# xyg-coder/min_llm_inference

Measured on AMD Instinct MI355X. Metric: decode tokens/sec (whole node) on synthetic batch, higher is better.
Workload: dtype bf16; 1 GPU; c4: paged KV decode step (attention + greedy decoder head, n_new=0), 1024 rows/GPU, emb_dim 512, max_seq 4096, lengths U[1024,1550], bf16 pages and weights, fp32 accumulate; lean composition: what the layers run -- no scores / probabilities / emb_score materialised, chunks merged inside the scan launch; rows_per_gpu=1024, rows_total=1024, emb_dim=512, max_seq=4096, n_vocab=1024, parallelism=row-sharded replicas x1, all-gather of token ids

## Files before the change

min_llm_inference_amd/csrc/attention_scan.hip:

```cpp
#include <string>

#include "device_common.hpp"
#include "scan_plan.hpp"

namespace mli {

constexpr int kScanThreads = 256;
constexpr int kScanWaves = kScanThreads / kWave;
constexpr int kMaxChunkTokens = 1024;
constexpr int kMinChunkTokens = 64;

void set_bf16_native_mfma(int v);
void set_scan_merge(int v);
void set_gemm_panel(int v);
void set_scan_stream(int v);
void set_scan_stream_min(int v);
void set_stream_dyn_pct(int v);
void set_stream_granule(int v);
void set_scan_resident_mib(int v);
void set_gemm_split(int v);
void set_bf16_split(int v);
void set_prefill_fused(int v);
void set_gemm_tall_tiles(int v);
void set_fill_compact(int v);
void set_latest_compact(int v);

static thread_local int g_chunk_tokens = 0;
static thread_local int g_nt_loads = 2;
static thread_local int g_row_order = 1;

constexpr int kQktUnits = 16384;
constexpr int kSvUnits = 2048;
constexpr int kSvMaxChunkTokens = 512;

static int pick_chunk_tokens(int n_batch, int n_sequence, int min_units = kQktUnits, int max_ct = kMaxChunkTokens) {
    if (g_chunk_tokens) return g_chunk_tokens;
    int ct = max_ct;
    while (ct > kMinChunkTokens && (int64_t)n_batch * ceil_div_i(n_sequence, ct) < min_units) ct >>= 1;
    return ct;
}

template <bool NT>
__global__ __launch_bounds__(kScanThreads) void qkt_paged_kernel(
    const float* __restrict__ q, const float* const* __restrict__ page_table,
    const int* __restrict__ lengths, float* __restrict__ qkt, int S, int D, int ct, SoftmaxStats st) {
    extern __shared__ __align__(16) unsigned char smem_raw[];
    __shared__ float2 wave_stats[kScanWaves];
    const int b = blockIdx.x;
    const int L = lengths[b];
    const int s0 = blockIdx.y * ct;
    if (s0 >= L) return;

    const int W = S / kPage;
    const int D4 = D >> 2;
    const int s1 = min(s0 + ct, L);
    const int npages = (s1 - s0 + kPage - 1) / kPage;

    float4* q_sh = reinterpret_cast<float4*>(smem_raw);
    const float** ptr_sh = reinterpret_cast<const float**>(smem_raw + (size_t)D4 * 16);

    const float4* q4 = reinterpret_cast<const float4*>(q + (int64_t)b * D);
    for (int i = threadIdx.x; i < D4; i += kScanThreads) q_sh[i] = q4[i];
    for (int i = threadIdx.x; i < npages; i += kScanThreads)
        ptr_sh[i] = page_table[(int64_t)b * W + s0 / kPage + i];
    __syncthreads();

    const int lane = threadIdx.x & (kWave - 1);
    const int wave = threadIdx.x >> 6;
    const float scale = sqrtf((float)D);
    const int nj = (D4 + kWave - 1) / kWave;
    constexpr int TB = 8;

    float run_m = -INFINITY, run_l = 0.f;
    for (int pi = wave; pi < npages; pi += kScanWaves) {
        const float* page = wave_uniform(ptr_sh[pi]);
        const float* krow = page + D;
        float acc[16];
#pragma unroll
        for (int t = 0; t < 16; ++t) acc[t] = 0.f;
        for (int j = 0; j < nj; ++j) {
            const int i4 = lane + j * kWave;
            if (i4 < D4) {
                const float4 qv = q_sh[i4];
                const unsigned voff = (unsigned)i4 * 16u;
#pragma unroll
                for (int h = 0; h < 16 / TB; ++h) {
                    float4 kv[TB];
#pragma unroll
                    for (int t = 0; t < TB; ++t) {
                        const float* trow = krow + (int64_t)(h * TB + t) * 3 * D;
                        kv[t] = ldg4<NT>(byte_offset(trow, voff));
                    }
#pragma unroll
                    for (int t = 0; t < TB; ++t) acc[h * TB + t] = dot4(qv, kv[t], acc[h * TB + t]);
                }
            }
        }
        const float tot = wave_reduce16(acc, lane);
        const int s = s0 + pi * kPage + (lane >> 2);
        const bool writer = (lane & 3) == 0 && s < L;
        const float score = tot / scale;
        if (writer) qkt[(int64_t)b * S + s] = score;
        if (st.stats != nullptr) stats_accumulate(score, writer, run_m, run_l);
    }
    if (st.stats != nullptr) {
        if (lane == 0) wave_stats[wave] = make_float2(run_m, run_l);
        __syncthreads();
        if (threadIdx.x == 0) {
            float m = -INFINITY;
            for (int w = 0; w < kScanWaves; ++w) m = fmaxf(m, wave_stats[w].x);
            float l = 0.f;
            for (int w = 0; w < kScanWaves; ++w)
                if (wave_stats[w].x != -INFINITY) l += wave_stats[w].y * expf(wave_stats[w].x - m);
            st.stats[(int64_t)b * st.per_row + blockIdx.y] = make_float2(m, l);
        }
    }
}

__global__ __launch_bounds__(kScanThreads) void qkt_naive_kernel(
    const float* __restrict__ q, const float* __restrict__ kt, const int* __restrict__ lengths,
    float* __restrict__ qkt, int S, int D, SoftmaxStats st) {
    extern __shared__ __align__(16) unsigned char smem_raw[];
    float4 (*red)[kWave] = reinterpret_cast<float4 (*)[kWave]>(smem_raw);
    float* q_sh = reinterpret_cast<float*>(smem_raw + sizeof(float4) * kScanWaves * kWave);
    const int b = blockIdx.x;
    const int L = lengths[b];
    const int s0 = blockIdx.y * 256;
    if (s0 >= L) return;
    for (int i = threadIdx.x; i < D; i += kScanThreads) q_sh[i] = q[(int64_t)b * D + i];
    __syncthreads();

    const int lane = threadIdx.x & (kWave - 1);
    const int wave = threadIdx.x >> 6;
    const int s = s0 + lane * 4;
    const bool in_row = s < S && s < L;
    const float* base = kt + (int64_t)b * D * S + s;
    const int d_per_wave = (D + kScanWaves - 1) / kScanWaves;
    const int d0 = wave * d_per_wave;
    const int d1 = min(d0 + d_per_wave, D);
    float4 acc = make_float4(0.f, 0.f, 0.f, 0.f);
    if (in_row) {
        int d = d0;
        for (; d + 8 <= d1; d += 8) {
            float4 kv[8];
#pragma unroll
            for (int u = 0; u < 8; ++u) kv[u] = *reinterpret_cast<const float4*>(base + (int64_t)(d + u) * S);
#pragma unroll
            for (int u = 0; u < 8; ++u) axpy4(q_sh[d + u], kv[u], acc);
        }
        for (; d < d1; ++d) axpy4(q_sh[d], *reinterpret_cast<const float4*>(base + (int64_t)d * S), acc);
    }
    red[wave][lane] = acc;
    __syncthreads();
    if (wave == 0) {
        float v[4] = {0.f, 0.f, 0.f, 0.f};
        if (in_row) {
            float4 r = red[0][lane];
#pragma unroll
            for (int w = 1; w < kScanWaves; ++w) {
                r.x += red[w][lane].x; r.y += red[w][lane].y; r.z += red[w][lane].z; r.w += red[w][lane].w;
            }
            const float scale = sqrtf((float)D);
            float* out = qkt + (int64_t)b * S + s;
            v[0] = r.x / scale; v[1] = r.y / scale; v[2] = r.z / scale; v[3] = r.w / scale;
            if (s + 4 <= L) {
                *reinterpret_cast<float4*>(out) = make_float4(v[0], v[1], v[2], v[3]);
            } else {
                for (int u = 0; u < 4; ++u) if (s + u < L) out[u] = v[u];
            }
        }
        if (st.stats != nullptr) {
            float m = -INFINITY, l = 0.f;
#pragma unroll
            for (int u = 0; u < 4; ++u) stats_accumulate(v[u], in_row && s + u < L, m, l);
// ... 307 lines not shown
#undef MLI_QKT_LAUNCH
    return launch_status();
}

int launch_qkt_paged(const float* q, const float* const* page_table, const int* lengths, float* qkt,
                     int B, int S, int D, hipStream_t st) {
    return launch_qkt_paged_stats(q, page_table, lengths, qkt, B, S, D, kNoStats, st);
}

int launch_qkt_naive_stats(const float* q, const float* kt, const int* lengths, float* qkt, int B, int S, int D,
                           SoftmaxStats stats, hipStream_t st) {
    if (S % 4 != 0 || B <= 0) return MLI_ERR_BAD_ARG;
    hipLaunchKernelGGL(qkt_naive_kernel, dim3(B, ceil_div_i(S, 256)), dim3(kScanThreads),
                       sizeof(float4) * kScanWaves * kWave + (size_t)D * 4, st, q, kt, lengths, qkt, S, D, stats);
    return launch_status();
}

int launch_qkt_naive(const float* q, const float* kt, const int* lengths, float* qkt, int B, int S, int D,
                     hipStream_t st) {
    return launch_qkt_naive_stats(q, kt, lengths, qkt, B, S, D, kNoStats, st);
}

int launch_softmax(float* qkt, const int* lengths, int B, int S, hipStream_t st) {
    if (S % 4 != 0 || B <= 0) return MLI_ERR_BAD_ARG;
    hipLaunchKernelGGL(softmax_lengths_kernel, dim3(B), dim3(kScanThreads), 0, st, qkt, lengths, B, S);
    return launch_status();
}

int launch_softmax_v_naive(const float* probs, const float* v_cache, const int* lengths, float* out,
                           int B, int S, int D, void* ws, size_t ws_bytes, hipStream_t st) {
    if (B <= 0 || S <= 0 || D <= 0) return MLI_ERR_BAD_ARG;
    float* p = const_cast<float*>(probs);
    if (D % 4 == 0) return launch_softmax_v_impl<4, false>(p, v_cache, lengths, out, B, S, D, ws, ws_bytes, kNoStats, st);
    return launch_softmax_v_impl<1, false>(p, v_cache, lengths, out, B, S, D, ws, ws_bytes, kNoStats, st);
}

int launch_softmax_v_paged(const float* probs, const float* const* page_table, const int* lengths, float* out,
                           int B, int S, int D, void* ws, size_t ws_bytes, hipStream_t st) {
    if (S % kPage != 0 || D % 4 != 0 || B <= 0) return MLI_ERR_BAD_ARG;
    return launch_softmax_v_impl<4, true>(const_cast<float*>(probs), page_table, lengths, out, B, S, D, ws, ws_bytes,
                                          kNoStats, st);
}

static thread_local int g_fused_softmax = -1;

static bool can_fuse(int B, int S, int stats_chunk, void* ws, size_t ws_bytes) {
    const bool want = g_fused_softmax == 1 || (g_fused_softmax < 0 && (int64_t)B * S <= (1 << 20));
    return want && ws != nullptr && ws_bytes >= stats_region_bytes(B, S) && ceil_div_i(S, stats_chunk) <= 256;
}

int launch_scores_softmax_v_paged(const float* q, const float* const* page_table, const int* lengths, float* qkt,
                                  float* out, int B, int S, int D, void* ws, size_t ws_bytes, hipStream_t st) {
    if (!can_fuse(B, S, pick_chunk_tokens(B, S), ws, ws_bytes)) {
        int rc = launch_qkt_paged(q, page_table, lengths, qkt, B, S, D, st);
        if (!rc) rc = launch_softmax(qkt, lengths, B, S, st);
        if (!rc) rc = launch_softmax_v_paged(qkt, page_table, lengths, out, B, S, D, ws, ws_bytes, st);
        return rc;
    }
    const SoftmaxStats stats = stats_view(ws, B, S, pick_chunk_tokens(B, S));
    int rc = launch_qkt_paged_stats(q, page_table, lengths, qkt, B, S, D, stats, st);
    if (rc) return rc;
    return launch_softmax_v_impl<4, true>(qkt, page_table, lengths, out, B, S, D, ws, ws_bytes, stats, st);
}

int launch_scores_softmax_v_naive(const float* q, const float* kt, const float* v_cache, const int* lengths,
                                  float* qkt, float* out, int B, int S, int D, void* ws, size_t ws_bytes,
                                  hipStream_t st) {
    if (!can_fuse(B, S, 256, ws, ws_bytes)) {
        int rc = launch_qkt_naive(q, kt, lengths, qkt, B, S, D, st);
        if (!rc) rc = launch_softmax(qkt, lengths, B, S, st);
        if (!rc) rc = launch_softmax_v_naive(qkt, v_cache, lengths, out, B, S, D, ws, ws_bytes, st);
        return rc;
    }
    const SoftmaxStats stats = stats_view(ws, B, S, 256);
    int rc = launch_qkt_naive_stats(q, kt, lengths, qkt, B, S, D, stats, st);
    if (rc) return rc;
    if (D % 4 == 0) return launch_softmax_v_impl<4, false>(qkt, v_cache, lengths, out, B, S, D, ws, ws_bytes, stats, st);
    return launch_softmax_v_impl<1, false>(qkt, v_cache, lengths, out, B, S, D, ws, ws_bytes, stats, st);
}

static size_t partial_region_bytes(int B, int S, int D) {
    const size_t nchunk = (size_t)ceil_div_i(S, kMinChunkTokens);
    return nchunk <= 1 ? 0 : (size_t)B * nchunk * (size_t)D * sizeof(float);
}
int fused_softmax_wanted(int B, int S) {
    return g_fused_softmax == 1 || (g_fused_softmax < 0 && (int64_t)B * S <= (1 << 20));
}

}

extern "C" {

size_t mli_attention_workspace_bytes(int n_batch, int n_sequence, int dim) {
    if (n_batch <= 0 || n_sequence <= 0 || dim <= 0) return 0;
    return mli::kArrivalRegionBytes + mli::stats_region_bytes(n_batch, n_sequence) +
           mli::partial_region_bytes(n_batch, n_sequence, dim);
}

int mli_attention_workspace_init(void* workspace, size_t workspace_bytes, void* stream) {
    if (workspace == nullptr || workspace_bytes < mli::kArrivalRegionBytes) return MLI_ERR_WORKSPACE;
    return (int)hipMemsetAsync(workspace, 0, mli::kArrivalRegionBytes, mli::as_stream(stream));
}

int mli_qkt(const float* q_output, const float* kt_cache, const int* lengths, float* qkt_output,
            int n_batch, int n_sequence, int dim, void* stream) {
    return mli::launch_qkt_naive(q_output, kt_cache, lengths, qkt_output, n_batch, n_sequence, dim,
                                 mli::as_stream(stream));
}

int mli_softmax_in_place_with_lengths(float* qkt_output, const int* lengths, int n_batch, int n_sequence,
                                      void* stream) {
    return mli::launch_softmax(qkt_output, lengths, n_batch, n_sequence, mli::as_stream(stream));
}

int mli_softmax_v(const float* softmax_result, const float* v_cache, const int* lengths, float* attention_result,
                  int n_batch, int n_sequence, int output_dim, void* workspace, size_t workspace_bytes,
                  void* stream) {
    { const mli::WsBody body = mli::ws_body(workspace, workspace_bytes); workspace = body.ptr; workspace_bytes = body.bytes; }
    return mli::launch_softmax_v_naive(softmax_result, v_cache, lengths, attention_result, n_batch, n_sequence,
                                       output_dim, workspace, workspace_bytes, mli::as_stream(stream));
}

int mli_qkt_paged(const float* q_output, const float* const* page_table, const int* lengths, float* qkt_output,
                  int n_batch, int n_sequence, int emb_dim, void* stream) {
    return mli::launch_qkt_paged(q_output, page_table, lengths, qkt_output, n_batch, n_sequence, emb_dim,
                                 mli::as_stream(stream));
}

int mli_softmax_v_paged(const float* softmax_result, const float* const* page_table, const int* lengths,
                        float* attention_result, int n_batch, int n_sequence, int emb_dim, void* workspace,
                        size_t workspace_bytes, void* stream) {
    { const mli::WsBody body = mli::ws_body(workspace, workspace_bytes); workspace = body.ptr; workspace_bytes = body.bytes; }
    return mli::launch_softmax_v_paged(softmax_result, page_table, lengths, attention_result, n_batch, n_sequence,
                                       emb_dim, workspace, workspace_bytes, mli::as_stream(stream));
}

int mli_tune(const char* key, int value) {
    const std::string k(key ? key : "");
    if (k == "chunk_tokens") {
        if (value != 0 && (value < mli::kMinChunkTokens || value > mli::kMaxChunkTokens || (value & (value - 1)))) return MLI_ERR_BAD_ARG;
        mli::g_chunk_tokens = value;
    } else if (k == "nt_loads") {
        mli::g_nt_loads = value < 0 || value > 2 ? 2 : value;
    } else if (k == "latest_compact") {
        mli::set_latest_compact(value);
    } else if (k == "fill_compact") {
        mli::set_fill_compact(value);
    } else if (k == "gemm_panel") {
        mli::set_gemm_panel(value);
    } else if (k == "gemm_tall_tiles") {
        mli::set_gemm_tall_tiles(value);
    } else if (k == "gemm_bf16_split") {
        mli::set_bf16_split(value);
    } else if (k == "prefill_fused") {
        mli::set_prefill_fused(value);
    } else if (k == "scan_row_order") {
        mli::g_row_order = value != 0;
    } else if (k == "gemm_split") {
        mli::set_gemm_split(value);
    } else if (k == "scan_stream") {
        mli::set_scan_stream(value);
    } else if (k == "scan_stream_dynamic_pct") {
        mli::set_stream_dyn_pct(value);
    } else if (k == "scan_stream_granule") {
        mli::set_stream_granule(value);
    } else if (k == "scan_resident_mib") {
        mli::set_scan_resident_mib(value);
    } else if (k == "scan_stream_min_tokens") {
        mli::set_scan_stream_min(value);
    } else if (k == "scan_merge") {
        mli::set_scan_merge(value);
    } else if (k == "fused_softmax") {
        mli::g_fused_softmax = value < 0 ? -1 : (value != 0);
    } else if (k == "bf16_native_mfma") {
        mli::set_bf16_native_mfma(value);
    } else {
        return MLI_ERR_BAD_ARG;
    }
    return 0;
}

int mli_stream_copy(const float* src, float* dst, size_t n_floats, void* stream) {
    if (n_floats % 4 != 0) return MLI_ERR_BAD_ARG;
    hipLaunchKernelGGL(mli::stream_copy_kernel, dim3(256 * 16), dim3(mli::kScanThreads), 0, mli::as_stream(stream),
                       reinterpret_cast<const float4*>(src), reinterpret_cast<float4*>(dst), n_floats / 4);
    return mli::launch_status();
}

int mli_stream_read(const float* src, float* sink, size_t n_floats, void* stream) {
    const size_t f4_per_wave = 4096;
    if (n_floats % (4 * f4_per_wave) != 0) return MLI_ERR_BAD_ARG;
    hipLaunchKernelGGL(mli::stream_read_kernel, dim3(256 * 8), dim3(mli::kScanThreads), 0, mli::as_stream(stream),
                       reinterpret_cast<const float4*>(src), sink, n_floats / 4, f4_per_wave);
    return mli::launch_status();
}

}
```

min_llm_inference_amd/csrc/proj_gemm_bf16.hip:

```cpp
#include <atomic>
#include <cstdlib>

#include "gemm_common.hpp"

namespace mli {

constexpr int HM = 64, HN = 64;
constexpr int kLdbBytes = HN * 2 + 64;
constexpr int kHThreads = 256;

int fill_compact(int n_new);
int latest_compact(int n_batch, int k_dim);
bool gemm_use_tall_tiles(int64_t tall_workgroups);

typedef __bf16 bf16x8_t __attribute__((ext_vector_type(8)));
typedef short s16x4_t __attribute__((ext_vector_type(4)));
typedef float f32x16_t __attribute__((ext_vector_type(16)));
typedef __attribute__((address_space(3))) s16x4_t* lds_s16x4_ptr;

#ifdef MLI_GEMM_TRACE
constexpr int kGemmTraceWgs = 1024;
__device__ unsigned long long mli_gemm_trace[kGemmTraceWgs * 8];
#define MLI_GT(var) const unsigned long long var = clock64()
#define MLI_GT_ADD(i, a, b) do { if (threadIdx.x == 0) gt_acc[i] += (b) - (a); } while (0)
#else
#define MLI_GT(var) do { } while (0)
#define MLI_GT_ADD(i, a, b) do { } while (0)
#endif

union Frag8 {
    bf16x8_t v;
    uint4 u;
    s16x4_t h[2];
};

template <int MODE_, int MT = 1, int KB = 32, bool FP8 = false>
__global__ __launch_bounds__(kHThreads) void gemm_bf16_mfma_kernel(GemmArgs g) {
    constexpr bool WIN = MODE_ == kPagedFillLive;
    constexpr int MODE = WIN ? kPagedFill : MODE_;
    constexpr int HM = 64 * MT;
    constexpr int HK = KB;
    constexpr int kLdaBytes = HK * 2 + 16;
    constexpr int AP = HM * HK / (kHThreads * 8);
    constexpr int BP = HK * HN / (kHThreads * 8);
    constexpr int kAThreadsPerRow = HK / 8;
    __shared__ __align__(16) unsigned char As[HM * kLdaBytes];
    __shared__ __align__(16) unsigned char Bs[HK * kLdbBytes];
    __shared__ const float* a_ptr[HM];
    __shared__ float* o_ptr[HM];
    constexpr bool kFillMode = MODE == kPagedFill;
    __shared__ const float* e_ptr[kFillMode ? HM : 1];
    __shared__ const float* p_ptr[kFillMode ? HM : 1];

    const int tiles_n = (g.N + HN - 1) / HN;
    const int wsel = blockIdx.x / tiles_n;
    const int n0 = (blockIdx.x % tiles_n) * HN;
    const int m0 = blockIdx.y * HM;
    const int z = blockIdx.z;
    const int out_id = g.out_id[wsel];
    const uint16_t* __restrict__ W = reinterpret_cast<const uint16_t*>(g.w[wsel]);

    constexpr bool kLatest = MODE == kPagedLatest;
    __shared__ FillIndex fill_index[1];
    const int tid = threadIdx.x;
    int fill_total = 0;
    if (g.compact) {
        fill_total = build_fill_index<kHThreads, kLatest, WIN>(g, fill_index[0]);
        if (m0 >= fill_total) return;
    } else if (MODE == kPagedFill && m0 >= g.lengths[g.new_batch_idx[z]]) {
        return;
    } else if (MODE == kPagedFill && WIN && fill_tile_dead(g, m0, HM, z)) {
        return;
    }
    const bool embed = kFillMode && g.emb_table != nullptr;
    if (tid < HM) {
        RowDesc r{nullptr, nullptr, nullptr, nullptr};
        if (g.compact) {
            if (m0 + tid < fill_total) {
                int zz, ss;
                if (WIN) fill_index_lookup_live(g, fill_index[0], m0 + tid, zz, ss);
                else fill_index_lookup(fill_index[0], kLatest ? g.B : g.n_new, m0 + tid, zz, ss);
                r = kLatest ? resolve_row<MODE, true, FP8>(g, zz, 0, out_id) : resolve_row<MODE, true, FP8>(g, ss, zz, out_id);
            }
        } else if (!WIN || !fill_token_dead(g, m0 + tid, z)) {
            r = resolve_row<MODE, true, FP8>(g, m0 + tid, z, out_id);
        }
        a_ptr[tid] = r.a;
        o_ptr[tid] = r.o;
        if (kFillMode) {
            e_ptr[tid] = r.e;
            p_ptr[tid] = r.p;
        }
    }
    __syncthreads();

    const int lane = tid & 63;
    const int wave = tid >> 6;
    const int wm = (wave >> 1) * 32 * MT;
    const int wn = (wave & 1) * 32;

    const int a_row = tid / kAThreadsPerRow, a_k8 = (tid % kAThreadsPerRow) * 8;
    constexpr int kARowsPerPass = kHThreads / kAThreadsPerRow;
    const int b_row = tid >> 3, b_n8 = (tid & 7) * 8;
    uint4 a_reg[AP], b_reg[BP];
    const uint16_t* a_src[AP];
    const float* e_src[AP];
    const float* p_src[AP];
#pragma unroll
    for (int p = 0; p < AP; ++p) {
        a_src[p] = reinterpret_cast<const uint16_t*>(a_ptr[a_row + p * kARowsPerPass]);
        e_src[p] = kFillMode ? e_ptr[a_row + p * kARowsPerPass] : nullptr;
        p_src[p] = kFillMode ? p_ptr[a_row + p * kARowsPerPass] : nullptr;
    }
    const bool writes_x = blockIdx.x == 0;

    auto load_tile = [&](int k0) {
#pragma unroll
        for (int p = 0; p < AP; ++p) {
            a_reg[p] = make_uint4(0, 0, 0, 0);
            if (kFillMode && embed && a_src[p] != nullptr) {
                if (k0 + a_k8 < g.K) {
                    const float4 e0 = *reinterpret_cast<const float4*>(e_src[p] + k0 + a_k8);
                    const float4 e1 = *reinterpret_cast<const float4*>(e_src[p] + k0 + a_k8 + 4);
                    const float4 p0 = *reinterpret_cast<const float4*>(p_src[p] + k0 + a_k8);
                    const float4 p1 = *reinterpret_cast<const float4*>(p_src[p] + k0 + a_k8 + 4);
                    if constexpr (FP8) {
                        const uint2 x8 = make_uint2(f32x4_to_fp8x4(e0.x + p0.x, e0.y + p0.y, e0.z + p0.z, e0.w + p0.w),
                                                    f32x4_to_fp8x4(e1.x + p1.x, e1.y + p1.y, e1.z + p1.z, e1.w + p1.w));
                        const uint2 lo = fp8x4_to_bf16x4(x8.x), hi = fp8x4_to_bf16x4(x8.y);
                        a_reg[p] = make_uint4(lo.x, lo.y, hi.x, hi.y);
                        if (writes_x)
                            *reinterpret_cast<uint2*>(const_cast<uint8_t*>(reinterpret_cast<const uint8_t*>(a_src[p])) + k0 + a_k8) = x8;
                    } else {
                        uint4 x;
                        x.x = f32_to_bf16(e0.x + p0.x) | ((uint32_t)f32_to_bf16(e0.y + p0.y) << 16);
                        x.y = f32_to_bf16(e0.z + p0.z) | ((uint32_t)f32_to_bf16(e0.w + p0.w) << 16);
                        x.z = f32_to_bf16(e1.x + p1.x) | ((uint32_t)f32_to_bf16(e1.y + p1.y) << 16);
                        x.w = f32_to_bf16(e1.z + p1.z) | ((uint32_t)f32_to_bf16(e1.w + p1.w) << 16);
                        a_reg[p] = x;
                        if (writes_x) *reinterpret_cast<uint4*>(const_cast<uint16_t*>(a_src[p]) + k0 + a_k8) = x;
                    }
                }
            } else if (a_src[p] != nullptr && k0 + a_k8 < g.K) {
                if constexpr (FP8) {
                    const uint2 x8 = *reinterpret_cast<const uint2*>(reinterpret_cast<const uint8_t*>(a_src[p]) + k0 + a_k8);
                    const uint2 lo = fp8x4_to_bf16x4(x8.x), hi = fp8x4_to_bf16x4(x8.y);
                    a_reg[p] = make_uint4(lo.x, lo.y, hi.x, hi.y);
                } else {
                    a_reg[p] = *reinterpret_cast<const uint4*>(a_src[p] + k0 + a_k8);
                }
            }
        }
#pragma unroll
        for (int p = 0; p < BP; ++p) {
            b_reg[p] = make_uint4(0, 0, 0, 0);
            const int k = k0 + b_row + p * 32, n = n0 + b_n8;
            if (k < g.K && n < g.N) b_reg[p] = *reinterpret_cast<const uint4*>(W + (int64_t)k * g.N + n);
        }
    };
    auto store_tile = [&]() {
#pragma unroll
        for (int p = 0; p < AP; ++p)
            *reinterpret_cast<uint4*>(&As[(a_row + p * kARowsPerPass) * kLdaBytes + a_k8 * 2]) = a_reg[p];
#pragma unroll
        for (int p = 0; p < BP; ++p)
            *reinterpret_cast<uint4*>(&Bs[(b_row + p * 32) * kLdbBytes + b_n8 * 2]) = b_reg[p];
    };

    f32x16_t acc[MT];
#pragma unroll
    for (int mt = 0; mt < MT; ++mt)
#pragma unroll
        for (int i = 0; i < 16; ++i) acc[mt][i] = 0.f;

    const int li = lane & 31, lh = lane >> 5;
    const unsigned a_off = (unsigned)((wm + li) * kLdaBytes + lh * 16);
    const int grp_col = wn + 16 * ((lane >> 4) & 1);
    const int tq = (lane >> 2) & 3, tp = lane & 3;
    const unsigned b_off = (unsigned)((8 * lh + tq) * kLdbBytes + (grp_col + 4 * tp) * 2);

    const int nk = (g.K + HK - 1) / HK;
#ifdef MLI_GEMM_TRACE
    unsigned long long gt_acc[5] = {0, 0, 0, 0, 0};
    const unsigned long long gt_begin = clock64();
#endif
    load_tile(0);
    store_tile();
    __syncthreads();
    for (int t = 0; t < nk; ++t) {
        MLI_GT(g0);
        if (t + 1 < nk) load_tile((t + 1) * HK);
        MLI_GT(g1);
        MLI_GT_ADD(0, g0, g1);
#pragma unroll
        for (int kk = 0; kk < HK; kk += 16) {
            Frag8 b;
            b.h[0] = __builtin_amdgcn_ds_read_tr16_b64_v4i16((lds_s16x4_ptr)(&Bs[b_off + kk * kLdbBytes]));
            b.h[1] = __builtin_amdgcn_ds_read_tr16_b64_v4i16((lds_s16x4_ptr)(&Bs[b_off + (kk + 4) * kLdbBytes]));
#pragma unroll
            for (int mt = 0; mt < MT; ++mt) {
                Frag8 a;
                a.u = *reinterpret_cast<const uint4*>(&As[a_off + mt * 32 * kLdaBytes + kk * 2]);
                acc[mt] = __builtin_amdgcn_mfma_f32_32x32x16_bf16(a.v, b.v, acc[mt], 0, 0, 0);
            }
        }
        MLI_GT(g2);
        MLI_GT_ADD(1, g1, g2);
        __syncthreads();
        MLI_GT(g3);
        MLI_GT_ADD(2, g2, g3);
        if (t + 1 < nk) {
            store_tile();
            MLI_GT(g4);
            MLI_GT_ADD(3, g3, g4);
            __syncthreads();
            MLI_GT(g5);
            MLI_GT_ADD(4, g4, g5);
        }
    }
#ifdef MLI_GEMM_TRACE
    {
        const unsigned wg = blockIdx.x + gridDim.x * blockIdx.y;
        if (threadIdx.x == 0 && wg < (unsigned)kGemmTraceWgs) {
            for (int i = 0; i < 5; ++i) mli_gemm_trace[wg * 8 + i] = gt_acc[i];
            mli_gemm_trace[wg * 8 + 5] = clock64() - gt_begin;
            mli_gemm_trace[wg * 8 + 6] = gt_begin;
            mli_gemm_trace[wg * 8 + 7] = (unsigned long long)nk;
        }
    }
#endif

#pragma unroll
    for (int mt = 0; mt < MT; ++mt) {
#pragma unroll
        for (int r = 0; r < 16; ++r) {
            const int mi = wm + mt * 32 + (r & 3) + 8 * (r >> 2) + 4 * lh;
            const int n = n0 + wn + li;
            float* op = o_ptr[mi];
            if (op != nullptr && n < g.N) {
                if (out_id == 1) op[n] = acc[mt][r];
                else if (FP8) reinterpret_cast<uint8_t*>(op)[n] = (uint8_t)f32_to_fp8(acc[mt][r]);
                else reinterpret_cast<uint16_t*>(op)[n] = f32_to_bf16(acc[mt][r]);
            }
        }
    }
}

constexpr int kDmThreads = 512;
constexpr int kDmM = 128, kDmK = 64;
constexpr int kDmABytes = kDmM * kDmK * 2;
constexpr int kDmSubBytes = kDmK * 64 * 2;
constexpr int kDmStageBytes = kDmABytes + 3 * kDmSubBytes;
constexpr int kDmStages = 3;
constexpr int kDmLoadsPerWave = (kDmStageBytes / 1024) / 4;
constexpr int kDmOutSubBytes = kDmM * 64 * 4;
constexpr size_t kDmSmem = (size_t)kDmStages * kDmStageBytes + kDmM * sizeof(void*);
static_assert(3 * kDmOutSubBytes <= kDmStages * kDmStageBytes, "the output tile reuses the stages");

#ifdef MLI_DMA_TRACE
constexpr int kDmaTraceWgs = 1024;
__device__ unsigned long long mli_dma_trace[kDmaTraceWgs * 16];
#define MLI_DT(var) const unsigned long long var = clock64()
#define MLI_DT_PUT(i, v) do { if (blockIdx.x < (unsigned)kDmaTraceWgs) mli_dma_trace[blockIdx.x * 16 + (i)] = (v); } while (0)
#else
#define MLI_DT(var) do { } while (0)
#define MLI_DT_PUT(i, v) do { } while (0)
#endif

typedef __attribute__((address_space(3))) void* lds_void_ptr;
typedef __attribute__((address_space(1))) void* global_void_ptr;

__device__ __forceinline__ void dma16(const unsigned char* src, unsigned char* lds_dst) {
    __builtin_amdgcn_global_load_lds((global_void_ptr)src, (lds_void_ptr)lds_dst, 16, 0, 0);
}

template <int MODE>
__global__ __launch_bounds__(kDmThreads) void gemm_bf16_dma_kernel(GemmArgs g, int col_tiles, int row_tiles) {
    static_assert(MODE == kPagedLatest, "decode projection only");
    extern __shared__ __align__(16) unsigned char dm_smem[];
    const uint16_t** a_ptr = reinterpret_cast<const uint16_t**>(dm_smem + kDmStages * kDmStageBytes);

    int ct, rt;
    if (col_tiles % 8 == 0) {
        const int xcd = blockIdx.x & 7, idx = blockIdx.x >> 3, cpx = col_tiles >> 3;
        rt = idx / cpx;
        ct = xcd * cpx + idx % cpx;
    } else {
        rt = blockIdx.x / col_tiles;
        ct = blockIdx.x % col_tiles;
    }
    (void)row_tiles;
    const int m0 = rt * kDmM;
    const int subs_per_w = g.N >> 6;
    const int tid = threadIdx.x;
    const int lane = tid & 63;
    const int wave = __builtin_amdgcn_readfirstlane(tid >> 6);
    const int nk = g.K / kDmK;
    MLI_DT(dt_entry);
#ifdef MLI_DMA_TRACE
    const unsigned long long dt_wall0 = wall_clock64();
#endif

    if (wave >= 4) {
        const int lw = wave - 4;
        const int r8 = lane >> 3, c8 = lane & 7;
        const unsigned char* src[kDmLoadsPerWave];
        int dst[kDmLoadsPerWave];
        const int64_t b_step = (int64_t)kDmK * g.N * 2;
#pragma unroll
        for (int i = 0; i < 6; ++i) {
            const int idx = lw * 6 + i;
            const int sub = idx >> 3, kb = (idx & 7) * 8;
            const int k = kb + r8;
            const int sg = ct * 3 + sub;
            const unsigned char* W = reinterpret_cast<const unsigned char*>(g.w[sg / subs_per_w]);
            src[i] = W + ((int64_t)k * g.N + (sg % subs_per_w) * 64) * 2 + ((c8 ^ (((k >> 1) & 1) << 2)) << 4);
            dst[i] = kDmABytes + sub * kDmSubBytes + kb * 128;
        }
        auto issue_b = [&](int t) {
            unsigned char* stage = dm_smem + (t % kDmStages) * kDmStageBytes;
#pragma unroll
            for (int i = 0; i < 6; ++i) {
                dma16(src[i], stage + dst[i]);
                src[i] += b_step;
            }
        };
        auto issue_a = [&](int t) {
            unsigned char* stage = dm_smem + (t % kDmStages) * kDmStageBytes;
#pragma unroll
            for (int i = 6; i < kDmLoadsPerWave; ++i) {
                dma16(src[i], stage + dst[i]);
                src[i] += kDmK * 2;
            }
        };
        issue_b(0);
        if (nk > 1) issue_b(1);
        __builtin_amdgcn_s_barrier();
        asm volatile("" ::: "memory");
#pragma unroll
        for (int i = 0; i < 4; ++i) {
            const int row = 32 * lw + 8 * i + r8;
            const uint16_t* p = a_ptr[row];
            if (p == nullptr) p = reinterpret_cast<const uint16_t*>(g.w[0]);
            src[6 + i] = reinterpret_cast<const unsigned char*>(p) + ((c8 ^ ((row >> 1) & 7)) << 4);
            dst[6 + i] = (32 * lw + 8 * i) * 128;
        }
        issue_a(0);
        if (nk > 1) issue_a(1);
#ifdef MLI_DMA_TRACE
        unsigned long long dt_wait = 0, dt_bar = 0, dt_issue = 0;
#endif
        for (int t = 0; t < nk; ++t) {
            MLI_DT(l0);
#ifdef MLI_DMA_TRACE
            if (g.n_new & 1) asm volatile("s_waitcnt vmcnt(0)" ::: "memory");
#endif
            if (t + 1 >= nk) asm volatile("s_waitcnt vmcnt(0)" ::: "memory");
            else if (t == 0) asm volatile("s_waitcnt vmcnt(4)" ::: "memory");
            else asm volatile("s_waitcnt vmcnt(%0)" ::"n"(kDmLoadsPerWave) : "memory");
            MLI_DT(l1);
            __builtin_amdgcn_s_barrier();
            asm volatile("" ::: "memory");
            MLI_DT(l2);
#ifdef MLI_DMA_TRACE
            if (g.n_new & 1) continue;
#endif
            if (t + 2 < nk) {
                issue_b(t + 2);
                issue_a(t + 2);
            }
#ifdef MLI_DMA_TRACE
            const unsigned long long l3 = clock64();
            dt_wait += l1 - l0; dt_bar += l2 - l1; dt_issue += l3 - l2;
#endif
        }
#ifdef MLI_DMA_TRACE
        if (tid == 256) { MLI_DT_PUT(8, dt_wait); MLI_DT_PUT(9, dt_bar); MLI_DT_PUT(10, dt_issue); }
#endif
        __builtin_amdgcn_s_barrier();
        __builtin_amdgcn_s_barrier();
        __builtin_amdgcn_s_barrier();
        asm volatile("" ::: "memory");
    } else {
// ... 10 lines not shown
#pragma unroll
                for (int i = 0; i < 16; ++i) acc[mt][nt][i] = 0.f;
        const int li = lane & 31, lh = lane >> 5;
        const int a_sw = (li >> 1) & 7;
        const unsigned a_row_off = (unsigned)((wm + li) * 128);
        const int tq = (lane >> 2) & 3, tp = lane & 3, g16 = (lane >> 4) & 1;
        unsigned b_off[3];
#pragma unroll
        for (int nt = 0; nt < 3; ++nt) {
            const int col = wn + nt * 32;
            b_off[nt] = (unsigned)(kDmABytes + (col >> 6) * kDmSubBytes + (8 * lh + tq) * 128 +
                                   ((((col >> 5) & 1) * 64 + g16 * 32 + tp * 8) ^ (((tq >> 1) & 1) << 6)));
        }
        auto read_frags = [&](const unsigned char* st, int q, Frag8 (&a)[2], Frag8 (&b)[3]) {
            const unsigned ac = (unsigned)(((2 * q + lh) ^ a_sw) << 4);
            a[0].u = *reinterpret_cast<const uint4*>(&st[a_row_off + ac]);
#pragma unroll
            for (int nt = 0; nt < 3; ++nt) {
                b[nt].h[0] = __builtin_amdgcn_ds_read_tr16_b64_v4i16((lds_s16x4_ptr)(&st[b_off[nt] + q * 16 * 128]));
                b[nt].h[1] = __builtin_amdgcn_ds_read_tr16_b64_v4i16((lds_s16x4_ptr)(&st[b_off[nt] + (q * 16 + 4) * 128]));
            }
            a[1].u = *reinterpret_cast<const uint4*>(&st[a_row_off + 32 * 128 + ac]);
        };
        auto multiply = [&](const Frag8 (&a)[2], const Frag8 (&b)[3]) {
#pragma unroll
            for (int mt = 0; mt < 2; ++mt)
#pragma unroll
                for (int nt = 0; nt < 3; ++nt)
                    acc[mt][nt] = __builtin_amdgcn_mfma_f32_32x32x16_bf16(a[mt].v, b[nt].v, acc[mt][nt], 0, 0, 0);
        };
        auto interleave = [&]() {
#pragma unroll
            for (int i = 0; i < 4; ++i) {
                __builtin_amdgcn_sched_group_barrier(0x008, 1, 0);
                __builtin_amdgcn_sched_group_barrier(0x100, 2, 0);
            }
            __builtin_amdgcn_sched_group_barrier(0x008, 2, 0);
        };
        Frag8 fa[3][2], fb[3][3];
        __syncthreads();
        MLI_DT(dt_first);
#ifdef MLI_DMA_TRACE
        unsigned long long dt_mbar = 0;
#endif
        read_frags(dm_smem, 0, fa[0], fb[0]);
        read_frags(dm_smem, 1, fa[1], fb[1]);
        for (int t0 = 0; t0 < nk; t0 += 3) {
#pragma unroll
            for (int j = 0; j < 3; ++j) {
                const int t = t0 + j;
                if (t < nk) {
                    const unsigned char* st = dm_smem + j * kDmStageBytes;
                    const unsigned char* nx = dm_smem + ((j + 1) % 3) * kDmStageBytes;
#pragma unroll
                    for (int q = 0; q < 4; ++q) {
                        const int cur = (4 * j + q) % 3, ahead = (4 * j + q + 2) % 3;
                        if (q == 2) {
                            MLI_DT(m0t);
                            __syncthreads();
#ifdef MLI_DMA_TRACE
                            dt_mbar += clock64() - m0t;
#endif
                        }
                        read_frags(q < 2 ? st : nx, (q + 2) & 3, fa[ahead], fb[ahead]);
                        multiply(fa[cur], fb[cur]);
                        interleave();
                    }
                }
            }
        }
        MLI_DT(dt_loop_end);
#ifdef MLI_DMA_TRACE
        if (tid == 0) {
            MLI_DT_PUT(0, dt_entry); MLI_DT_PUT(1, dt_rows); MLI_DT_PUT(2, dt_first); MLI_DT_PUT(3, dt_loop_end);
            MLI_DT_PUT(5, dt_mbar);
        }
#endif
        __syncthreads();
#ifdef MLI_DMA_TRACE
        if (tid == 0) MLI_DT_PUT(11, clock64());
#endif
#pragma unroll
        for (int nt = 0; nt < 3; ++nt) {
            const int col = wn + nt * 32;
            unsigned char* C = dm_smem + (col >> 6) * kDmOutSubBytes + (((col >> 5) & 1) * 32 + li) * 4;
#pragma unroll
            for (int mt = 0; mt < 2; ++mt)
#pragma unroll
                for (int r = 0; r < 16; ++r)
                    *reinterpret_cast<float*>(&C[(wm + mt * 32 + (r & 3) + 8 * (r >> 2) + 4 * lh) * 256]) = acc[mt][nt][r];
        }
        __syncthreads();
#ifdef MLI_DMA_TRACE
        if (tid == 0) MLI_DT_PUT(12, clock64());
#endif
    }

    const uint16_t* q_row[4];
    const uint16_t* kv_row[2];
#pragma unroll
    for (int i = 0; i < 4; ++i) q_row[i] = a_ptr[wave * 16 + i * 4 + (lane >> 4)];
#pragma unroll
    for (int i = 0; i < 2; ++i) kv_row[i] = a_ptr[wave * 16 + i * 8 + (lane >> 3)];
    auto load_sub = [&](int sub, uint4 (&v)[4]) -> int {
        const int out_id = g.out_id[(ct * 3 + sub) / subs_per_w];
        const unsigned char* C = dm_smem + sub * kDmOutSubBytes;
        if (out_id == 1) {
#pragma unroll
            for (int i = 0; i < 4; ++i)
                v[i] = *reinterpret_cast<const uint4*>(&C[(wave * 16 + i * 4 + (lane >> 4)) * 256 + (lane & 15) * 16]);
        } else {
#pragma unroll
            for (int i = 0; i < 4; ++i)
                v[i] = *reinterpret_cast<const uint4*>(&C[(wave * 16 + (i >> 1) * 8 + (lane >> 3)) * 256 + (lane & 7) * 32 + (i & 1) * 16]);
        }
        return out_id;
    };
    auto pack2 = [](uint32_t a, uint32_t b) { return (uint32_t)f32_to_bf16(__uint_as_float(a)) | ((uint32_t)f32_to_bf16(__uint_as_float(b)) << 16); };
    typedef unsigned int u32x4_t __attribute__((ext_vector_type(4)));
    typedef __attribute__((address_space(1))) u32x4_t* global_u32x4_ptr;
    auto store_sub = [&](int sub, int out_id, const uint4 (&v)[4]) {
        const int n = ((ct * 3 + sub) % subs_per_w) * 64;
        if (out_id == 1) {
#pragma unroll
            for (int i = 0; i < 4; ++i) {
                const int row = wave * 16 + i * 4 + (lane >> 4);
                if (q_row[i] != nullptr)
                    *(global_u32x4_ptr)(g.q_output + (int64_t)(m0 + row) * g.N + n + (lane & 15) * 4) = u32x4_t{v[i].x, v[i].y, v[i].z, v[i].w};
            }
        } else {
            const int64_t seg = (int64_t)(out_id == 0 ? kSegK : kSegV) * g.K;
#pragma unroll
            for (int i = 0; i < 2; ++i) {
                const u32x4_t w{pack2(v[2 * i].x, v[2 * i].y), pack2(v[2 * i].z, v[2 * i].w),
                                pack2(v[2 * i + 1].x, v[2 * i + 1].y), pack2(v[2 * i + 1].z, v[2 * i + 1].w)};
                if (kv_row[i] != nullptr) *(global_u32x4_ptr)(const_cast<uint16_t*>(kv_row[i]) + seg + n + (lane & 7) * 8) = w;
            }
        }
    };
    uint4 v0[4], v1[4], v2[4];
    const int o0 = load_sub(0, v0), o1 = load_sub(1, v1), o2 = load_sub(2, v2);
    store_sub(0, o0, v0);
    store_sub(1, o1, v1);
    store_sub(2, o2, v2);
#ifdef MLI_DMA_TRACE
    if (tid == 0) MLI_DT_PUT(13, clock64());
    asm volatile("s_waitcnt vmcnt(0)" ::: "memory");
    if (tid == 0) { MLI_DT_PUT(4, clock64()); MLI_DT_PUT(6, wall_clock64() - dt_wall0); }
#endif
}

static thread_local int g_bf16_split = 1;
void set_bf16_split(int v) { g_bf16_split = v != 0; }

int launch_latest_paged_bf16_native(uint16_t* const* page_table, const int* lengths, const uint16_t* wk,
                                    const uint16_t* wq, const uint16_t* wv, float* q, int B, int S, int D,
                                    hipStream_t st) {
    GemmArgs g{};
    g.w[0] = reinterpret_cast<const float*>(wk); g.w[1] = reinterpret_cast<const float*>(wq);
    g.w[2] = reinterpret_cast<const float*>(wv); g.n_out = 3;
    g.out_id[0] = 0; g.out_id[1] = 1; g.out_id[2] = 2;
    g.M = B; g.N = D; g.K = D;
    g.page_table = reinterpret_cast<float* const*>(page_table); g.q_output = q; g.lengths = lengths;
    g.B = B; g.S = S;
    g.compact = latest_compact(B, D);
    const int tiles_x = ceil_div_i(D, HN) * 3;
    if (g_bf16_split && D % 64 == 0 && gemm_use_tall_tiles((int64_t)1 << 40) && (D >= 1536 || (D >= 1024 && B >= 320))) {
        static std::atomic<unsigned long long> dma_opted_in{0};
        int device = 0;
        (void)hipGetDevice(&device);
        const unsigned long long bit = 1ull << (device & 63);
        if (!(dma_opted_in.load(std::memory_order_relaxed) & bit)) {
            hipError_t e = hipFuncSetAttribute(reinterpret_cast<const void*>(&gemm_bf16_dma_kernel<kPagedLatest>),
                                               hipFuncAttributeMaxDynamicSharedMemorySize, (int)kDmSmem);
            if (e != hipSuccess) return (int)e;
            dma_opted_in.fetch_or(bit, std::memory_order_relaxed);
        }
        g.compact = 0;
#ifdef MLI_DMA_TRACE
        if (const char* dbg = std::getenv("MLI_DMA_DEBUG")) g.n_new = std::atoi(dbg);
#endif
        const int col_tiles = D / 64, row_tiles = ceil_div_i(B, kDmM);
        hipLaunchKernelGGL((gemm_bf16_dma_kernel<kPagedLatest>), dim3(col_tiles * row_tiles), dim3(kDmThreads), kDmSmem, st,
                           g, col_tiles, row_tiles);
        return launch_status();
    }
    if (gemm_use_tall_tiles((int64_t)tiles_x * ceil_div_i(B, 128))) {
        hipLaunchKernelGGL((gemm_bf16_mfma_kernel<kPagedLatest, 2, 64>), dim3(tiles_x, ceil_div_i(B, 128), 1),
                           dim3(kHThreads), 0, st, g);
        return launch_status();
    }
    dim3 grid(tiles_x, ceil_div_i(B, HM), 1);
    if (D >= 256 && D <= 1024)
        hipLaunchKernelGGL((gemm_bf16_mfma_kernel<kPagedLatest, 1, 128>), grid, dim3(kHThreads), 0, st, g);
    else
        hipLaunchKernelGGL((gemm_bf16_mfma_kernel<kPagedLatest>), grid, dim3(kHThreads), 0, st, g);
    return launch_status();
}

template <bool FP8, bool WIN>
static int fill_paged_16bit_embed(const float* emb_table, const float* wpe, const int* tokens, void* const* page_table,
                                  const int* new_idx, const int* lengths, const uint16_t* wk, const uint16_t* wv, int B, int S,
                                  int D, int n_new, int window, int n_sink, hipStream_t st) {
    if (n_new == 0) return 0;
    if (n_new < 0 || B <= 0 || S % kPage != 0 || D % (FP8 ? 16 : 8) != 0) return MLI_ERR_BAD_ARG;
    GemmArgs g{};
    g.emb_table = emb_table; g.wpe = wpe; g.inp = tokens;
    g.w[0] = reinterpret_cast<const float*>(wk); g.w[1] = reinterpret_cast<const float*>(wv); g.n_out = 2;
    g.out_id[0] = 0; g.out_id[1] = 2;
    g.M = S; g.N = D; g.K = D;
    g.page_table = reinterpret_cast<float* const*>(page_table); g.lengths = lengths; g.new_batch_idx = new_idx;
    g.B = B; g.S = S;
    g.n_new = n_new; g.compact = fill_compact(n_new);
    if (WIN) { g.fill_window = window; g.fill_sink = n_sink; }
    const int flat_rows = WIN ? live_tokens_bound(S, window, n_sink) : S;
    dim3 grid(ceil_div_i(D, HN) * 2, ceil_div_i(S, HM), n_new);
    if (g.compact) grid = dim3(ceil_div_i(D, HN) * 2, ceil_div_i(flat_rows * n_new, HM), 1);
    hipLaunchKernelGGL((gemm_bf16_mfma_kernel<WIN ? kPagedFillLive : kPagedFill, 1, 32, FP8>), grid, dim3(kHThreads), 0, st, g);
    return launch_status();
}

int launch_fill_paged_bf16_embed(const float* emb_table, const float* wpe, const int* tokens,
                                 uint16_t* const* page_table, const int* new_idx, const int* lengths, const uint16_t* wk,
                                 const uint16_t* wv, int B, int S, int D, int n_new, hipStream_t st) {
    return fill_paged_16bit_embed<false, false>(emb_table, wpe, tokens, reinterpret_cast<void* const*>(page_table), new_idx,
                                                lengths, wk, wv, B, S, D, n_new, 0, 0, st);
}

int launch_fill_paged_bf16_window_embed(const float* emb_table, const float* wpe, const int* tokens,
                                        uint16_t* const* page_table, const int* new_idx, const int* lengths,
                                        const uint16_t* wk, const uint16_t* wv, int B, int S, int D, int n_new, int window,
                                        int n_sink, hipStream_t st) {
    return fill_paged_16bit_embed<false, true>(emb_table, wpe, tokens, reinterpret_cast<void* const*>(page_table), new_idx,
                                               lengths, wk, wv, B, S, D, n_new, window, n_sink, st);
}

int launch_latest_paged_fp8(uint8_t* const* page_table, const int* lengths, const uint16_t* wk, const uint16_t* wq,
                            const uint16_t* wv, float* q, int B, int S, int D, hipStream_t st) {
    if (B <= 0 || S % kPage != 0 || D % 16 != 0) return MLI_ERR_BAD_ARG;
    GemmArgs g{};
    g.w[0] = reinterpret_cast<const float*>(wk); g.w[1] = reinterpret_cast<const float*>(wq);
    g.w[2] = reinterpret_cast<const float*>(wv); g.n_out = 3;
    g.out_id[0] = 0; g.out_id[1] = 1; g.out_id[2] = 2;
    g.M = B; g.N = D; g.K = D;
    g.page_table = reinterpret_cast<float* const*>(page_table); g.q_output = q; g.lengths = lengths;
    g.B = B; g.S = S;
    g.compact = latest_compact(B, D);
    const int tiles_x = ceil_div_i(D, HN) * 3;
    if (gemm_use_tall_tiles((int64_t)tiles_x * ceil_div_i(B, 128))) {
        hipLaunchKernelGGL((gemm_bf16_mfma_kernel<kPagedLatest, 2, 64, true>), dim3(tiles_x, ceil_div_i(B, 128), 1),
                           dim3(kHThreads), 0, st, g);
        return launch_status();
    }
    dim3 grid(tiles_x, ceil_div_i(B, HM), 1);
    if (D >= 256 && D <= 1024)
        hipLaunchKernelGGL((gemm_bf16_mfma_kernel<kPagedLatest, 1, 128, true>), grid, dim3(kHThreads), 0, st, g);
    else
        hipLaunchKernelGGL((gemm_bf16_mfma_kernel<kPagedLatest, 1, 32, true>), grid, dim3(kHThreads), 0, st, g);
    return launch_status();
}

int launch_fill_paged_fp8_embed(const float* emb_table, const float* wpe, const int* tokens, uint8_t* const* page_table,
                                const int* new_idx, const int* lengths, const uint16_t* wk, const uint16_t* wv, int B, int S,
                                int D, int n_new, hipStream_t st) {
    return fill_paged_16bit_embed<true, false>(emb_table, wpe, tokens, reinterpret_cast<void* const*>(page_table), new_idx,
                                               lengths, wk, wv, B, S, D, n_new, 0, 0, st);
}

int launch_fill_paged_fp8_window_embed(const float* emb_table, const float* wpe, const int* tokens,
                                       uint8_t* const* page_table, const int* new_idx, const int* lengths, const uint16_t* wk,
                                       const uint16_t* wv, int B, int S, int D, int n_new, int window, int n_sink,
                                       hipStream_t st) {
    return fill_paged_16bit_embed<true, true>(emb_table, wpe, tokens, reinterpret_cast<void* const*>(page_table), new_idx,
                                              lengths, wk, wv, B, S, D, n_new, window, n_sink, st);
}

int launch_fill_paged_bf16_native(uint16_t* const* page_table, const int* new_idx, const int* lengths,
                                  const uint16_t* wk, const uint16_t* wv, int B, int S, int D, int n_new,
                                  hipStream_t st) {
    return launch_fill_paged_bf16_embed(nullptr, nullptr, nullptr, page_table, new_idx, lengths, wk, wv, B, S, D, n_new, st);
}

}

#ifdef MLI_DMA_TRACE
extern "C" int mli_debug_dma_trace(unsigned long long* host, int n_wgs) {
    if (n_wgs > mli::kDmaTraceWgs) n_wgs = mli::kDmaTraceWgs;
    return (int)hipMemcpyFromSymbol(host, HIP_SYMBOL(mli::mli_dma_trace), (size_t)n_wgs * 16 * sizeof(unsigned long long));
}
#endif

#ifdef MLI_GEMM_TRACE
extern "C" int mli_debug_gemm_trace(unsigned long long* host, int n_wgs) {
    if (n_wgs > mli::kGemmTraceWgs) n_wgs = mli::kGemmTraceWgs;
    return (int)hipMemcpyFromSymbol(host, HIP_SYMBOL(mli::mli_gemm_trace), (size_t)n_wgs * 8 * sizeof(unsigned long long));
}
#endif
```

Measured before the change: 1.244 million tokens/s.

## Preload whole-K weights and activations into registers for decode QKV projection

Adds a whole-K path for the decode-time latest-token projection GEMM with D of 256, 384 or 512. The whole B weight panel is loaded into registers before the fill-index and row-resolution work, and all A slices are loaded ahead of compute. The kernel then runs double-buffered 64-wide K stages in LDS with lighter lgkm-only barriers. The aim is to hide global-load latency behind setup and remove the per-K-step load/sync loop, at the cost of much higher register pressure and possible occupancy loss.

```diff
diff --git a/min_llm_inference_amd/csrc/attention_scan.hip b/min_llm_inference_amd/csrc/attention_scan.hip
--- a/min_llm_inference_amd/csrc/attention_scan.hip
+++ b/min_llm_inference_amd/csrc/attention_scan.hip
@@ -20,6 +20,7 @@
 void set_scan_resident_mib(int v);
 void set_gemm_split(int v);
 void set_bf16_split(int v);
+void set_proj_whole_k(int v);
 void set_prefill_fused(int v);
 void set_gemm_tall_tiles(int v);
 void set_fill_compact(int v);
@@ -633,6 +634,8 @@
         mli::set_gemm_tall_tiles(value);
     } else if (k == "gemm_bf16_split") {
         mli::set_bf16_split(value);
+    } else if (k == "proj_whole_k") {
+        mli::set_proj_whole_k(value);
     } else if (k == "prefill_fused") {
         mli::set_prefill_fused(value);
     } else if (k == "scan_row_order") {
diff --git a/min_llm_inference_amd/csrc/proj_gemm_bf16.hip b/min_llm_inference_amd/csrc/proj_gemm_bf16.hip
--- a/min_llm_inference_amd/csrc/proj_gemm_bf16.hip
+++ b/min_llm_inference_amd/csrc/proj_gemm_bf16.hip
@@ -16,6 +16,10 @@
 typedef __bf16 bf16x8_t __attribute__((ext_vector_type(8)));
 typedef short s16x4_t __attribute__((ext_vector_type(4)));
 typedef float f32x16_t __attribute__((ext_vector_type(16)));
+typedef unsigned wk_u32x4_t __attribute__((ext_vector_type(4)));
+typedef unsigned wk_u32x2_t __attribute__((ext_vector_type(2)));
+typedef const __attribute__((address_space(1))) wk_u32x4_t* wk_global_x4_ptr;
+typedef const __attribute__((address_space(1))) wk_u32x2_t* wk_global_x2_ptr;
 typedef __attribute__((address_space(3))) s16x4_t* lds_s16x4_ptr;
 
 #ifdef MLI_GEMM_TRACE
@@ -34,18 +38,35 @@
     s16x4_t h[2];
 };
 
-template <int MODE_, int MT = 1, int KB = 32, bool FP8 = false>
+__device__ __forceinline__ void lds_barrier() {
+    asm volatile("s_waitcnt lgkmcnt(0)" ::: "memory");
+    __builtin_amdgcn_s_barrier();
+    asm volatile("" ::: "memory");
+}
+
+template <int N, int I = 0, class F>
+__device__ __forceinline__ void unrolled(F&& f) {
+    if constexpr (I < N) {
+        f(std::integral_constant<int, I>{});
+        unrolled<N, I + 1>(static_cast<F&&>(f));
+    }
+}
+
+template <int MODE_, int MT = 1, int KB = 32, bool FP8 = false, int NK = 0>
 __global__ __launch_bounds__(kHThreads) void gemm_bf16_mfma_kernel(GemmArgs g) {
     constexpr bool WIN = MODE_ == kPagedFillLive;
     constexpr int MODE = WIN ? kPagedFill : MODE_;
+    constexpr bool WK = NK > 0;
+    static_assert(!WK || (MODE_ == kPagedLatest && MT == 1 && KB == 128 && NK <= 4), "whole K: the 64 x 64, KB = 128 decode launch");
     constexpr int HM = 64 * MT;
-    constexpr int HK = KB;
+    constexpr int HK = WK ? 64 : KB;
+    constexpr int kStages = WK ? 2 : 1;
     constexpr int kLdaBytes = HK * 2 + 16;
     constexpr int AP = HM * HK / (kHThreads * 8);
     constexpr int BP = HK * HN / (kHThreads * 8);
     constexpr int kAThreadsPerRow = HK / 8;
-    __shared__ __align__(16) unsigned char As[HM * kLdaBytes];
-    __shared__ __align__(16) unsigned char Bs[HK * kLdbBytes];
+    __shared__ __align__(16) unsigned char As[kStages * HM * kLdaBytes];
+    __shared__ __align__(16) unsigned char Bs[kStages * HK * kLdbBytes];
     __shared__ const float* a_ptr[HM];
     __shared__ float* o_ptr[HM];
     constexpr bool kFillMode = MODE == kPagedFill;
@@ -63,6 +84,15 @@
     constexpr bool kLatest = MODE == kPagedLatest;
     __shared__ FillIndex fill_index[1];
     const int tid = threadIdx.x;
+    const int b_row = tid >> 3, b_n8 = (tid & 7) * 8;
+    constexpr int NH = WK ? 2 * NK : 1;
+    wk_u32x4_t wk_b[NH][BP];
+    if constexpr (WK) {
+        unrolled<NH * BP>([&](auto I) {
+            constexpr int h = decltype(I)::value / BP, p = decltype(I)::value % BP;
+            wk_b[h][p] = *(wk_global_x4_ptr)(W + (int64_t)(h * HK + b_row + p * 32) * g.N + n0 + b_n8);
+        });
+    }
     int fill_total = 0;
     if (g.compact) {
         fill_total = build_fill_index<kHThreads, kLatest, WIN>(g, fill_index[0]);
@@ -92,7 +122,8 @@
             p_ptr[tid] = r.p;
         }
     }
-    __syncthreads();
+    if constexpr (WK) lds_barrier();
+    else __syncthreads();
 
     const int lane = tid & 63;
     const int wave = tid >> 6;
@@ -101,7 +132,6 @@
 
     const int a_row = tid / kAThreadsPerRow, a_k8 = (tid % kAThreadsPerRow) * 8;
     constexpr int kARowsPerPass = kHThreads / kAThreadsPerRow;
-    const int b_row = tid >> 3, b_n8 = (tid & 7) * 8;
     uint4 a_reg[AP], b_reg[BP];
     const uint16_t* a_src[AP];
     const float* e_src[AP];
@@ -179,6 +209,46 @@
     const int tq = (lane >> 2) & 3, tp = lane & 3;
     const unsigned b_off = (unsigned)((8 * lh + tq) * kLdbBytes + (grp_col + 4 * tp) * 2);
 
+    if constexpr (WK) {
+        using XRaw = std::conditional_t<FP8, wk_u32x2_t, wk_u32x4_t>;
+        XRaw wk_a[NH][AP];
+#pragma unroll
+        for (int p = 0; p < AP; ++p)
+            if (a_src[p] == nullptr) a_src[p] = W;
+        unrolled<NH * AP>([&](auto I) {
+            constexpr int h = decltype(I)::value / AP, p = decltype(I)::value % AP;
+            if constexpr (FP8) wk_a[h][p] = *(wk_global_x2_ptr)(reinterpret_cast<const uint8_t*>(a_src[p]) + h * HK + a_k8);
+            else wk_a[h][p] = *(wk_global_x4_ptr)(a_src[p] + h * HK + a_k8);
+        });
+        unrolled<NH>([&](auto H) {
+            constexpr int h = decltype(H)::value;
+            unsigned char* as = As + (h & 1) * (HM * kLdaBytes);
+            unsigned char* bs = Bs + (h & 1) * (HK * kLdbBytes);
+#pragma unroll
+            for (int p = 0; p < AP; ++p) {
+                wk_u32x4_t x;
+                if constexpr (FP8) {
+                    const uint2 lo = fp8x4_to_bf16x4(wk_a[h][p].x), hi = fp8x4_to_bf16x4(wk_a[h][p].y);
+                    x = wk_u32x4_t{lo.x, lo.y, hi.x, hi.y};
+                } else {
+                    x = wk_a[h][p];
+                }
+                *reinterpret_cast<wk_u32x4_t*>(&as[(a_row + p * kARowsPerPass) * kLdaBytes + a_k8 * 2]) = x;
+            }
+#pragma unroll
+            for (int p = 0; p < BP; ++p)
+                *reinterpret_cast<wk_u32x4_t*>(&bs[(b_row + p * 32) * kLdbBytes + b_n8 * 2]) = wk_b[h][p];
+            lds_barrier();
+#pragma unroll
+            for (int kk = 0; kk < HK; kk += 16) {
+                Frag8 a, b;
+                b.h[0] = __builtin_amdgcn_ds_read_tr16_b64_v4i16((lds_s16x4_ptr)(&bs[b_off + kk * kLdbBytes]));
+                b.h[1] = __builtin_amdgcn_ds_read_tr16_b64_v4i16((lds_s16x4_ptr)(&bs[b_off + (kk + 4) * kLdbBytes]));
+                a.u = *reinterpret_cast<const uint4*>(&as[a_off + kk * 2]);
+                acc[0] = __builtin_amdgcn_mfma_f32_32x32x16_bf16(a.v, b.v, acc[0], 0, 0, 0);
+            }
+        });
+    } else {
     const int nk = (g.K + HK - 1) / HK;
 #ifdef MLI_GEMM_TRACE
     unsigned long long gt_acc[5] = {0, 0, 0, 0, 0};
@@ -229,6 +299,7 @@
         }
     }
 #endif
+    }
 
 #pragma unroll
     for (int mt = 0; mt < MT; ++mt) {
@@ -545,6 +616,21 @@
 
 static thread_local int g_bf16_split = 1;
 void set_bf16_split(int v) { g_bf16_split = v != 0; }
+
+static thread_local int g_proj_whole_k = 1;
+void set_proj_whole_k(int v) { g_proj_whole_k = v != 0; }
+
+template <bool FP8>
+static void launch_latest_kb128(const GemmArgs& g, dim3 grid, int D, hipStream_t st) {
+#ifndef MLI_GEMM_TRACE
+    if (g_proj_whole_k && D % 64 == 0) {
+        if (D == 256) { hipLaunchKernelGGL((gemm_bf16_mfma_kernel<kPagedLatest, 1, 128, FP8, 2>), grid, dim3(kHThreads), 0, st, g); return; }
+        if (D == 384) { hipLaunchKernelGGL((gemm_bf16_mfma_kernel<kPagedLatest, 1, 128, FP8, 3>), grid, dim3(kHThreads), 0, st, g); return; }
+        if (D == 512) { hipLaunchKernelGGL((gemm_bf16_mfma_kernel<kPagedLatest, 1, 128, FP8, 4>), grid, dim3(kHThreads), 0, st, g); return; }
+    }
+#endif
+    hipLaunchKernelGGL((gemm_bf16_mfma_kernel<kPagedLatest, 1, 128, FP8>), grid, dim3(kHThreads), 0, st, g);
+}
 
 int launch_latest_paged_bf16_native(uint16_t* const* page_table, const int* lengths, const uint16_t* wk,
                                     const uint16_t* wq, const uint16_t* wv, float* q, int B, int S, int D,
@@ -585,7 +671,7 @@
     }
     dim3 grid(tiles_x, ceil_div_i(B, HM), 1);
     if (D >= 256 && D <= 1024)
-        hipLaunchKernelGGL((gemm_bf16_mfma_kernel<kPagedLatest, 1, 128>), grid, dim3(kHThreads), 0, st, g);
+        launch_latest_kb128<false>(g, grid, D, st);
     else
         hipLaunchKernelGGL((gemm_bf16_mfma_kernel<kPagedLatest>), grid, dim3(kHThreads), 0, st, g);
     return launch_status();
@@ -647,7 +733,7 @@
     }
     dim3 grid(tiles_x, ceil_div_i(B, HM), 1);
     if (D >= 256 && D <= 1024)
-        hipLaunchKernelGGL((gemm_bf16_mfma_kernel<kPagedLatest, 1, 128, true>), grid, dim3(kHThreads), 0, st, g);
+        launch_latest_kb128<true>(g, grid, D, st);
     else
         hipLaunchKernelGGL((gemm_bf16_mfma_kernel<kPagedLatest, 1, 32, true>), grid, dim3(kHThreads), 0, st, g);
     return launch_status();
```

Measured after the change: 1.209 million tokens/s. -2.9%, worse.
